# ETHZ-RobotX/open3d_slam_advanced_rss_2024_public

Hardware: AMD Instinct MI355X
Metric: ICP iterations/s (100k-pt scan vs 2M-pt map) (higher is better)
Workload: dtype f32; 1 GPU; C2: 100000-pt scan vs 2000000-pt voxel map, 0.1 m voxels, 50 iters, icp.yaml chain (KDTree maxDist 0.5 exact, Trimmed 0.9, SurfaceNormal 1.57, PointToPlane); scan_points=100000, map_points=2000000, pairs_per_gpu=1, parallelism=1 independent scan/map pair, 1 per GPU, no data-path collective

## Files before the change

### open3d_slam_advanced_rss_2024_public_amd/csrc/icp_kernels.h

```cpp
#pragma once
#include <hip/hip_runtime.h>
#include <math.h>
#include <stdint.h>
#include "host_post.h"
#include "icp_types.h"
#include "solve_device.h"

#pragma clang fp contract(off)

namespace o3s {
namespace kern {

constexpr int kBlock = 256;

constexpr float kInfF = __builtin_huge_valf();

template <int CTRL>
__device__ __forceinline__ int dpp_i32(int v) {
  return __builtin_amdgcn_update_dpp(v, v, CTRL, 0xF, 0xF, false);
}
template <int CTRL>
__device__ __forceinline__ double dpp_f64(double v) {
  const int lo = dpp_i32<CTRL>(__double2loint(v)), hi = dpp_i32<CTRL>(__double2hiint(v));
  return __hiloint2double(hi, lo);
}
__device__ __forceinline__ double readlane_f64(double v, int lane) {
// ... 403 lines not shown
  uint32_t tot;
  uint32_t ex = block_excl_scan(s, &tot, sh) + sums[blockIdx.x];
#pragma unroll
  for (int k = 0; k < kScanItems; ++k) {
    if (base + k < n) out[base + k] = ex;
    ex += v[k];
  }
  if (base <= n - 1 && n - 1 < base + kScanItems) out[n] = ex;
}

constexpr int kMaxQTiles = 2048;
constexpr int kTileReplicas = 8;
__device__ __forceinline__ uint32_t qcount_slot(uint32_t lin) { return (lin & ~2047u) | ((lin & 63u) << 5) | ((lin >> 6) & 31u); }
static_assert(kScanTile == 2048, "qcount_slot transposes a 64 x 32 tile");
struct Mat16 {
  float v[16];
};
struct PrepInit {
  uint32_t* hist;
  int hist_words;
  uint32_t* sel;
  int sel_words;
  float4* mq;
  float* cert;
  IcpState* state;
  int seed_differential;
  uint32_t seq;
};

__global__ void __launch_bounds__(kBlock) k_read_prep(const float4* __restrict__ in_xyzw, const float* __restrict__ in_n ,
                                                      int N, Mat16 T0, GridParams g,
                                                      float* __restrict__ tx, float* __restrict__ ty, float* __restrict__ tz,
                                                      float* __restrict__ tnx, float* __restrict__ tny, float* __restrict__ tnz,
                                                      uint32_t* __restrict__ cell_of, uint32_t* __restrict__ counts ,
                                                      int qf, int qnx, int qny, PrepInit init,
                                                      uint32_t* __restrict__ ticket ,
                                                      uint32_t* __restrict__ tile_cnt ,
                                                      int32_t* __restrict__ perm ) {
  const int i = blockIdx.x * kBlock + threadIdx.x;
  if (init.hist) {
    const int stride = gridDim.x * kBlock;
    for (int k = i; k < init.hist_words; k += stride) init.hist[k] = 0u;
    for (int k = i; k < init.sel_words; k += stride) init.sel[k] = 0u;
    if (blockIdx.x == 0) {
      constexpr int kWords = (int)(sizeof(IcpState) / 4);
      uint32_t* w = reinterpret_cast<uint32_t*>(init.state);
      for (int k = threadIdx.x; k < kWords; k += kBlock) w[k] = 0u;
      __syncthreads();
      if (threadIdx.x == 0) {
        IcpState* S = init.state;
        S->T_iter[0] = S->T_iter[5] = S->T_iter[10] = S->T_iter[15] = 1.f;
        S->limit = kInfF;
        S->call_seq = init.seq;
        S->t_prep = wall_clock64();
        if (init.seed_differential) {
          S->quat_ring[0][3] = 1.f;
          S->hist_total = 1;
        }
      }
    }
  }
  __shared__ uint32_t s_tile[kMaxQTiles];
  if (counts) {
    for (int k = threadIdx.x; k < kMaxQTiles; k += kBlock) s_tile[k] = 0u;
    __syncthreads();
  }
  int my_tile = -1;
  if (i < N) {
    if (init.mq) init.mq[i] = make_float4(0.f, 0.f, 0.f, 0.f);
    if (init.cert) init.cert[i] = 0.f;
    const float4 p = in_xyzw[i];
    float T[16];
#pragma unroll
    for (int k = 0; k < 16; ++k) T[k] = T0.v[k];
    const float x = xf_row(T, 0, p.x, p.y, p.z), y = xf_row(T, 1, p.x, p.y, p.z), z = xf_row(T, 2, p.x, p.y, p.z);
    tx[i] = x;
    ty[i] = y;
    tz[i] = z;
    if (in_n) {
      const float a = in_n[3 * i], b = in_n[3 * i + 1], c = in_n[3 * i + 2];
      tnx[i] = rot_row(T, 0, a, b, c);
      tny[i] = rot_row(T, 1, a, b, c);
      tnz[i] = rot_row(T, 2, a, b, c);
    }
    if (counts) {
      const int cx = cell_coord(x, g.ox, g.inv_cell, g.nx);
      const int cy = cell_coord(y, g.oy, g.inv_cell, g.ny);
      const int cz = cell_coord(z, g.oz, g.inv_cell, g.nz);
      const uint32_t lin = ((uint32_t)(cz / qf) * (uint32_t)qny + (uint32_t)(cy / qf)) * (uint32_t)qnx + (uint32_t)(cx / qf);
      cell_of[i] = lin;
      ticket[i] = atomicAdd(&counts[qcount_slot(lin)], 1u);
      const int tile = (int)(lin / (uint32_t)kScanTile);
      if (atomicAdd(&s_tile[tile], 1u) == 0u) my_tile = tile;
// ... 196 lines not shown
    d = c ? od : d;
    idx = c ? oi : idx;
  }
  gd = d;
  gi = idx;
}

constexpr int kFarMaxCells = 4096;

constexpr int kFarWaves = 5;
constexpr int kFarQ = 6;
template <bool STATS, int G, int UN, int RCB, bool FAR, bool CERT>
__global__ void __launch_bounds__(kBlock, FAR ? kFarWaves : 7) k_match2(const float* __restrict__ rx, const float* __restrict__ ry, const float* __restrict__ rz,
                                                      int N, const float4* __restrict__ ref, const uint32_t* __restrict__ cell_start,
                                                      GridParams g, IcpState* __restrict__ st,
                                                      int32_t* __restrict__ pos_out, float* __restrict__ d2_out, float4* __restrict__ mq,
                                                      uint32_t* __restrict__ hist_rep,
                                                      const float4* __restrict__ refn ,
                                                      float4* __restrict__ mn ,
                                                      const float* __restrict__ rnx, const float* __restrict__ rny,
                                                      const float* __restrict__ rnz ,
                                                      int rep_mask ,
                                                      uint32_t* __restrict__ spec ,
                                                      float* __restrict__ cert
                                                      O3S_DBG_PARAM
                                                      O3S_HOOK_PARAM(uint32_t* __restrict__ settled_cnt )) {
  __shared__ uint32_t s_hist[kHistBins];
  __shared__ uint32_t s_cnt[2];
  if (threadIdx.x < 2) s_cnt[threadIdx.x] = 0u;
#ifdef O3S_TEST_HOOKS
  __shared__ uint32_t s_set[2];
  if (threadIdx.x < 2) s_set[threadIdx.x] = 0u;
#endif
  constexpr int TQ = kBlock / G;
  constexpr int NK = (9 + G - 1) / G;
  const int sub = threadIdx.x & (G - 1);
  const int qib = threadIdx.x / G;
  const int tile = (blockIdx.x & 7) * (gridDim.x >> 3) + (blockIdx.x >> 3);
  const int i = tile * TQ + qib;
  const bool valid = i < N;
  const float hv = hdr_load(st);
  const float hp = CERT ? reinterpret_cast<const float*>(st->T_prev)[threadIdx.x & 31] : 0.f;
  float px = 0.f, py = 0.f, pz = 0.f;
  float4 inc = make_float4(0.f, 0.f, 0.f, 0.f);
  float cq = 0.f;
  int pe = -1;
  if (valid) {
    px = rx[i];
    py = ry[i];
    pz = rz[i];
    inc = mq[i];
    if (CERT) {
      cq = cert[i];
      pe = pos_out[i];
    }
  }
  for (int k = threadIdx.x; k < kHistBins; k += kBlock) s_hist[k] = 0u;
  if (hdr_i(hv, H_DONE)) return;
  if (blockIdx.x == 0) {
    for (int k = threadIdx.x; k < 1024; k += kBlock) hist_rep[(size_t)kHistReplicas * kHistBins + k] = 0u;
    if (threadIdx.x == 0 && hdr_i(hv, H_ITER) == 0) st->t_begin = wall_clock64();
    if (spec)
      for (int k = threadIdx.x; k < kSpecHalf; k += kBlock) spec[(size_t)((hdr_i(hv, H_ITER) + 1) & 1) * kSpecHalf + k] = 0u;
    if (CERT && threadIdx.x == 0) st->cert_seq[hdr_i(hv, H_ITER) & 1] = (uint32_t)hdr_i(hv, H_ITER) + 1u;
  }
  const uint32_t hint = __float_as_uint(hdr_f(hv, H_LIMIT));
  const bool spec_on = spec != nullptr && hdr_i(hv, H_ITER) > 0 && hint < 0x7f800000u;
  uint32_t* const spec_cur = spec_on ? spec + (size_t)(hdr_i(hv, H_ITER) & 1) * kSpecHalf : nullptr;
  float T[16];
#pragma unroll
  for (int k = 0; k < 16; ++k) T[k] = hdr_f(hv, k);
  __syncthreads();
  const float lim = g.max_r2;
  unsigned long long n_cand = 0, n_rows = 0;

  const float sx = xf_row(T, 0, px, py, pz), sy = xf_row(T, 1, px, py, pz), sz = xf_row(T, 2, px, py, pz);
// ... 2 lines not shown
  int gi = 0x7fffffff;
  bool active = valid && ((fabsf(sx) + fabsf(sy)) + fabsf(sz) < kInfF);
  float bound = lim;
  int mybin = -1;
  auto count_match = [&](float d) {
    const int bin = (int)((__float_as_uint(d) >> 20) & (kHistBins - 1));
    if (!O3S_DBG(1) && atomicAdd(&s_hist[bin], 1u) == 0u) mybin = bin;
    if (spec_on && !O3S_DBG(1)) {
      const uint32_t key = __float_as_uint(d) & 0x7fffffffu;
      if ((key >> 20) == (hint >> 20)) atomicAdd(&spec_cur[(key >> 10) & 1023u], 1u);
      if ((key >> 10) == (hint >> 10)) atomicAdd(&spec_cur[1024 + (key & 1023u)], 1u);
    }
  };
  uint32_t n_found = 0u, n_below = 0u;
  auto tally = [&](bool counted, float d) {
    if (spec_on && !O3S_DBG(1)) {
      const bool below = counted && ((__float_as_uint(d) & 0x7fffffffu) >> 20) < (hint >> 20);
      n_found += (uint32_t)__popcll(__ballot(counted));
      n_below += (uint32_t)__popcll(__ballot(below));
    }
  };
  bool wave_settled = false;
  bool settled = false;
  if (CERT) {
    float Tp[16];
#pragma unroll
    for (int k = 0; k < 16; ++k) Tp[k] = hdr_f(hp, k);
    float dn = 0.f, cn = 0.f;
    const bool fresh = (uint32_t)hdr_i(hp, 16 + ((hdr_i(hv, H_ITER) + 1) & 1)) == (uint32_t)hdr_i(hv, H_ITER);
    if (fresh && active && cq > 0.f) {
      const float ex = sx - xf_row(Tp, 0, px, py, pz), ey = sy - xf_row(Tp, 1, px, py, pz), ez = sz - xf_row(Tp, 2, px, py, pz);
      const float delta = __builtin_sqrtf((ex * ex + ey * ey) + ez * ez) * (1.f + 1e-6f);
      const float L = __builtin_sqrtf(cq) - delta;
      const float L2 = L * L, thr = L2 * (1.f - 1e-5f);
      cn = L2 * (1.f - 1e-6f);
      if (inc.w != 0.f) {
        dn = dist2(sx, sy, sz, inc.x, inc.y, inc.z);
        settled = (L > 0.f) & (pe != -1) & (dn <= lim) & (dn < thr);
      } else {
        settled = (L > 0.f) & (thr > lim);
      }
    }
    wave_settled = __all(!valid || settled);
#ifdef O3S_TEST_HOOKS
    if (settled_cnt && hdr_i(hv, H_ITER) < kSpecTrace) {
      const int n_set = __popcll(__ballot(settled && sub == 0));
      if ((threadIdx.x & 63) == 0 && n_set) {
        atomicAdd(&s_set[0], (uint32_t)n_set);
        if (wave_settled) atomicAdd(&s_set[1], (uint32_t)n_set);
      }
    }
#endif
    if (settled && !O3S_DBG(8)) {
      if (sub == 0) {
        if (inc.w != 0.f) {
          pos_out[i] = pe >= 0 ? pe : -2 - pe;
          d2_out[i] = dn;
          count_match(dn);
        }
        cert[i] = cn;
      }
    }
    tally(settled && !O3S_DBG(8) && sub == 0 && inc.w != 0.f, dn);
    active = active && !settled;
  }
  if (active) {
    const float di = dist2(sx, sy, sz, inc.x, inc.y, inc.z);
    bound = ((inc.w != 0.f) & (di <= lim)) ? di : lim;
  }
  float others = kInfF;
  auto group_cert = [&](float o) {
    float cn = (gi != 0x7fffffff && b.idx == gi) ? o : fminf(o, b.d);
    if (G >= 2) cn = fminf(cn, __int_as_float(dpp_i32<0xB1>(__float_as_int(cn))));
    if (G >= 4) cn = fminf(cn, __int_as_float(dpp_i32<0x4E>(__float_as_int(cn))));
    return ((fabsf(sx) + fabsf(sy)) + fabsf(sz) < kInfF) ? cn * (1.f - 1e-6f) : 0.f;
  };
  if (FAR && rnx != nullptr && lim * g.inv_cell * g.inv_cell >= 25.f && !wave_settled && __any(valid && !settled && inc.w == 0.f)) {
    constexpr int kProbeSteps = 12;
    constexpr int NP = (2 * kProbeSteps + G - 1) / G;
    const bool want = valid && !settled && inc.w == 0.f;
    float nx = 0.f, ny = 0.f, nz = 0.f;
    if (want) {
      const float a = rnx[i], b_ = rny[i], c_ = rnz[i];
      nx = rot_row(T, 0, a, b_, c_);
      ny = rot_row(T, 1, a, b_, c_);
      nz = rot_row(T, 2, a, b_, c_);
    }
    const int n_steps = min(kProbeSteps, (int)(__builtin_sqrtf(lim) * g.inv_cell) + 1);
    U32Pair hd[NP];
    int kk_[NP];
#pragma unroll
    for (int u = 0; u < NP; ++u) {
      const int e = sub + u * G;
      const int st_ = (e >> 1) + 1;
      const float t_ = (float)st_ * g.cell * ((e & 1) ? -1.f : 1.f);
      const float qx_ = sx + t_ * nx, qy_ = sy + t_ * ny, qz_ = sz + t_ * nz;
      const int cx_ = (int)floorf((qx_ - g.ox) * g.inv_cell), cy_ = (int)floorf((qy_ - g.oy) * g.inv_cell), cz_ = (int)floorf((qz_ - g.oz) * g.inv_cell);
      const bool in = want & (st_ <= n_steps) & ((unsigned)cx_ < (unsigned)g.nx) & ((unsigned)cy_ < (unsigned)g.ny) & ((unsigned)cz_ < (unsigned)g.nz);
// ... 24 lines not shown
    if (G >= 2) ds = fminf(ds, __int_as_float(dpp_i32<0xB1>(__float_as_int(ds))));
    if (G >= 4) ds = fminf(ds, __int_as_float(dpp_i32<0x4E>(__float_as_int(ds))));
    bound = fminf(bound, ds);
  }
  if (active) {
    const CellGeom c = cell_geom(sx, sy, sz, g);
    const float gxn = fmaxf(c.lx - g.margin, 0.f), gxp = fmaxf((g.cell - c.lx) - g.margin, 0.f);
    const float gyn = fmaxf(c.ly - g.margin, 0.f), gyp = fmaxf((g.cell - c.ly) - g.margin, 0.f);
    const float gzn = fmaxf(c.lz - g.margin, 0.f), gzp = fmaxf((g.cell - c.lz) - g.margin, 0.f);
    const float gxn2 = gxn * gxn, gxp2 = gxp * gxp, gyn2 = gyn * gyn, gyp2 = gyp * gyp, gzn2 = gzn * gzn, gzp2 = gzp * gzp;
    uint32_t jb[NK], len[NK];
    {
      uint4 w[NK];
      int span[NK];
      uint32_t inm[NK];
#pragma unroll
      for (int k = 0; k < NK; ++k) {
        const int t = sub + k * G, tt = t < 9 ? t : 4;
        const int dz = tt / 3 - 1, dy = tt % 3 - 1;
        const int z = c.cz + dz, y = c.cy + dy;
        const float gz2 = dz < 0 ? gzn2 : (dz > 0 ? gzp2 : 0.f);
        const float gy2 = dy < 0 ? gyn2 : (dy > 0 ? gyp2 : 0.f);
        const float g2 = gz2 + gy2;
        const float rem = bound - g2;
        const bool lskip = gxn2 > rem, rskip = gxp2 > rem;
        const int lo = max(c.cx - (int)!lskip, 0);
        const int hi = min(c.cx + (int)!rskip, g.nx - 1);
        const bool row = (t < 9) & ((unsigned)y < (unsigned)g.ny) & ((unsigned)z < (unsigned)g.nz);
        const bool in = row & (lo <= hi) & !(g2 > bound) & !O3S_DBG(4);
        const float ol = (lskip & ((unsigned)(c.cx - 1) < (unsigned)g.nx)) ? g2 + gxn2 : kInfF;
        const float orr = (rskip & ((unsigned)(c.cx + 1) < (unsigned)g.nx)) ? g2 + gxp2 : kInfF;
        others = row ? fminf(others, (g2 > bound) ? g2 : fminf(ol, orr)) : others;
        inm[k] = (uint32_t) - (int)in;
        span[k] = hi - lo;
        const uint32_t off = (((uint32_t)z * (uint32_t)g.ny + (uint32_t)y) * (uint32_t)g.nx + (uint32_t)lo) & inm[k];
        w[k] = *reinterpret_cast<const uint4*>(cell_start + off);
      }
#pragma unroll
      for (int k = 0; k < NK; ++k) {
        const uint32_t ve = span[k] == 0 ? w[k].y : (span[k] == 1 ? w[k].z : w[k].w);
        jb[k] = w[k].x & inm[k];
        len[k] = (ve - w[k].x) & inm[k];
        if (STATS) {
          n_rows += len[k] ? 1 : 0;
          n_cand += (unsigned long long)len[k];
        }
      }
    }
    uint32_t P[9], D[9];
    uint32_t total = 0;
#pragma unroll
    for (int t = 0; t < 9; ++t) {
      const uint32_t l_t = group_bcast_dyn<G>(len[t / G], t % G);
      const uint32_t j_t = group_bcast_dyn<G>(jb[t / G], t % G);
      P[t] = total;
// ... 5 lines not shown
      float4 qv[UN];
      uint32_t jj[UN];
      bool ok[UN];
#pragma unroll
      for (int u = 0; u < UN; ++u) {
        const uint32_t f = f0 + (uint32_t)(u * G);
        ok[u] = f < total;
        uint32_t dsel = D[0];
#pragma unroll
        for (int t = 1; t < 9; ++t) dsel = (P[t] <= f) ? D[t] : dsel;
        jj[u] = ok[u] ? f + dsel : 0u;
        qv[u] = ref[jj[u]];
      }
#pragma unroll
      for (int u = 0; u < UN; ++u) own_take(b, others, dist2(sx, sy, sz, qv[u].x, qv[u].y, qv[u].z), qv[u], (int)jj[u], lim, ok[u]);
    }
  }
  group_min_di<G>(b.d, b.idx, gd, gi);
  {
    const float q = g.cell - g.margin;
    const bool far = active && !(q * q > fminf(gd, bound)) && !O3S_DBG(16);
    if (active && !far) others = fminf(others, q * q);
    if (!FAR && CERT && valid && !settled && !O3S_DBG(8)) {
      const float cn = group_cert(far ? 0.f : others);
      if (sub == 0) cert[i] = cn;
    }
    active = far;
  }
  if (FAR) {
    if (__any(active)) {
      constexpr int Q = kFarQ;
      const CellGeom c = cell_geom(sx, sy, sz, g);
      const float m_yz = fminf(fminf(c.ly, g.cell - c.ly), fminf(c.lz, g.cell - c.lz));
      const int rho0 = max(max(0, max(-c.cy, c.cy - (g.ny - 1))), max(-c.cz, c.cz - (g.nz - 1)));
      const int rho_max = max(max(c.cy, g.ny - 1 - c.cy), max(c.cz, g.nz - 1 - c.cz));
      int rho = rho0;
      float best = fminf(gd, bound);
      auto ring_lb2_yz = [&](int r) {
        const float lb = (float)(r - 1) * g.cell + m_yz - g.margin;
        return (r >= 2 && lb > 0.f) ? lb * lb : 0.f;
      };
      if (active && rho <= rho_max && ring_lb2_yz(rho) > best) others = fminf(others, ring_lb2_yz(rho));
      if (rho > rho_max || ring_lb2_yz(rho) > best) active = false;
      uint32_t qa[Q], qb[Q];
#pragma unroll
      for (int k = 0; k < Q; ++k) qa[k] = qb[k] = 0u;
      while (__any(active)) {
// ... 173 lines not shown
#pragma unroll
                for (int v = 0; v < RCB; ++v) q[v] = ref[j + v < j1 ? j + v : j0];
#pragma unroll
                for (int v = 0; v < RCB; ++v) own_take(b, no_cert, dist2(sx, sy, sz, q[v].x, q[v].y, q[v].z), q[v], (int)(j + v), lim, j + v < j1);
              }
              if (STATS) {
                n_rows += j1 > j0 ? 1 : 0;
                n_cand += (unsigned long long)(j1 - j0);
              }
            }
          }
        }
      }
      group_min_di<G>(b.d, b.idx, gd, gi);
      if (active) {
        r += 1;
        if (r > rmax || ring_lb2(r, m, g) + extra2 > fminf(gd, bound)) active = false;
      }
    }
  }
  bool counted = false;
  if (valid && !settled && !O3S_DBG(8)) {
    const bool found = gi != 0x7fffffff;
    const float cn = (FAR && CERT) ? group_cert(others) : 0.f;
    bool mine = found && b.idx == gi && b.pos >= 0;
    if (FAR && G >= 2) {
      const uint32_t m = mine ? 1u : 0u;
      const uint32_t m0 = group_bcast<G, 0>(m), m1 = group_bcast<G, 1 % G>(m), m2 = group_bcast<G, 2 % G>(m);
      const bool lower = ((sub > 0) & (m0 != 0u)) | ((G >= 4) & (sub > 1) & (m1 != 0u)) | ((G >= 4) & (sub > 2) & (m2 != 0u));
      mine = mine && !lower;
    }
    if (mine) {
      const float4 nq = (mn && refn) ? refn[b.pos] : make_float4(0.f, 0.f, 0.f, 0.f);
      pos_out[i] = b.pos;
      d2_out[i] = b.d;
      mq[i] = make_float4(b.qx, b.qy, b.qz, 1.f);
      if (mn) mn[i] = nq;
      if (FAR && CERT) cert[i] = cn;
      count_match(b.d);
      counted = true;
    } else if (!found && sub == 0) {
      pos_out[i] = -1;
      d2_out[i] = kInfF;
      mq[i] = make_float4(0.f, 0.f, 0.f, 0.f);
      if (mn) mn[i] = make_float4(0.f, 0.f, 0.f, 0.f);
      if (FAR && CERT) cert[i] = cn;
    }
// ... 1395 lines not shown
  float p[3], q[3];
  const float4 nn = mn[i];
  cov_chain_pair(T, rx[i], ry[i], rz[i], mq[i], st->mp[0], st->mp[1], st->mp[2], st->mq[0], st->mq[1], st->mq[2], p, q);
  float* o = out + (size_t)i * 9;
  o[0] = p[0], o[1] = p[1], o[2] = p[2], o[3] = q[0], o[4] = q[1], o[5] = q[2], o[6] = nn.x, o[7] = nn.y, o[8] = nn.z;
  keep[i] = k ? 1 : 0;
}

__global__ void __launch_bounds__(kBlock) k_export_matches(int N, const int32_t* __restrict__ pos, const float* __restrict__ d2,
                                                           const float4* __restrict__ ref, const int32_t* __restrict__ perm,
                                                           int32_t* __restrict__ ids, float* __restrict__ dists) {
  const int i = blockIdx.x * kBlock + threadIdx.x;
  if (i >= N) return;
  const int pe = pos[i];
  const int o = perm[i];
  const int slot = pe >= 0 ? pe : (pe <= -2 ? -2 - pe : -1);
  ids[o] = slot >= 0 ? __float_as_int(ref[slot].w) : -1;
  dists[o] = d2[i];
}

__global__ void __launch_bounds__(kBlock) k_import_matches(int N, const int32_t* __restrict__ ids, const float* __restrict__ dists,
                                                           const float* __restrict__ weights , const int32_t* __restrict__ orig_to_sorted,
                                                           int64_t M, const float4* __restrict__ ref, int32_t* __restrict__ pos, float* __restrict__ d2,
                                                           float4* __restrict__ mq, float* __restrict__ cert ) {
  const int i = blockIdx.x * kBlock + threadIdx.x;
  if (i >= N) return;
  if (cert) cert[i] = 0.f;
  const int id = ids[i];
  const float d = dists[i];
  int pe = -1;
  if (id >= 0 && (int64_t)id < M) {
    pe = orig_to_sorted[id];
    if (weights && weights[i] == 0.0f) pe = -2 - pe;
  }
  float4 q = make_float4(0.f, 0.f, 0.f, 0.f);
  if (id >= 0 && (int64_t)id < M) {
    const float4 r = ref[orig_to_sorted[id]];
    q = make_float4(r.x, r.y, r.z, 1.f);
  }
  mq[i] = q;
  if (d == kInfF) pe = pe >= 0 ? -2 - pe : pe;
  pos[i] = pe;
  d2[i] = d;
}

__global__ void __launch_bounds__(kBlock) k_weights(int N, const int32_t* __restrict__ pos, const float* __restrict__ d2,
                                                    const float* __restrict__ read_n , const float4* __restrict__ refn,
                                                    ChainParams cp, const IcpState* __restrict__ st, int any_filter, float* __restrict__ w) {
  const int i = blockIdx.x * kBlock + threadIdx.x;
  if (i >= N) return;
// ... 37 lines not shown
```

### open3d_slam_advanced_rss_2024_public_amd/csrc/icp_types.h

```cpp
#pragma once
#include <stddef.h>
#include <stdint.h>
#include <hip/hip_runtime.h>

#ifdef O3S_TEST_HOOKS
#include <stdlib.h>
#define O3S_HOOK_ENV(name) getenv(name)
#define O3S_DBG_PARAM , int dbg
#define O3S_DBG_ARG(x) , (x)
#define O3S_HOOK_PARAM(decl) , decl
#define O3S_DBG(bits) ((dbg & (bits)) != 0)
#define O3S_CP_DBG(cp, bits) (((cp).dbg & (bits)) != 0)
#else
#define O3S_HOOK_ENV(name) ((const char*)0)
#define O3S_DBG_PARAM
#define O3S_DBG_ARG(x)
#define O3S_HOOK_PARAM(decl)
#define O3S_DBG(bits) false
#define O3S_CP_DBG(cp, bits) false
#endif

namespace o3s {

constexpr int kHistBins = 2048;
// ... 57 lines not shown
  float point_used_ratio, weighted_ratio;
  float A[36];
  float b[6];
  float x[6];
  float dT[16];
  float ang_ring[kHistRing];
  float tnorm_ring[kHistRing];
  uint32_t call_seq;
  uint32_t posted;
  unsigned long long t_begin;
  unsigned long long t_end;
  unsigned long long t_prep;
  unsigned long long cand_count;
  unsigned long long row_count;
  float T_prev[16];
  uint32_t cert_seq[2];
  uint32_t tail_pad[14];
};
constexpr int kStateWords = (int)(offsetof(IcpState, T_prev) / 4);
constexpr int kStateTailWords = 4;
static_assert(offsetof(IcpState, T_prev) == offsetof(IcpState, row_count) + 8, "the staged words end with the matcher's counters");
static_assert(sizeof(IcpState) % 4 == 0, "IcpState is copied word-wise");
static_assert(offsetof(IcpState, cert_seq) == offsetof(IcpState, T_prev) + 64 && sizeof(IcpState) == offsetof(IcpState, T_prev) + 128,
              "k_match2 loads T_prev and cert_seq as one 32-word block");

struct CandRec {
  float px, py, pz;
  uint32_t bits;
  float qx, qy, qz;
  int32_t keep;
};

struct SelScratch {
  uint32_t seg_count[kSegs];
  uint32_t bin;
  uint32_t kk;
  uint32_t bin_count;
  uint32_t skip;
  uint32_t reserved;
  uint32_t pad[3];
  uint32_t depth;
  uint32_t limit_bits;
  uint32_t pad2[2];
};
static_assert(sizeof(SelScratch) == 64, "the selection kernels read the hand-off words one per lane (lanes 0..15)");
constexpr int kSelWordDepth = 12, kSelWordLimit = 13;

// ... 10 lines not shown
```

### open3d_slam_advanced_rss_2024_public_amd/csrc/o3s_icp.hip

```cpp
#include "../../include/o3s_icp.h"

#include <hip/hip_runtime.h>

#include <algorithm>
#include <cmath>
#include <cstdio>
#include <cstdlib>
#include <cstring>
#include <limits>
#include <string>
#include <vector>

#include "icp_kernels.h"
#include "icp_shard_kernels.h"
#include "icp_types.h"

#pragma clang fp contract(off)

using namespace o3s;

namespace {

thread_local std::string g_create_error;

// ... 29 lines not shown
struct HostStage {
  IcpState state;
  IcpState eval_state;
  float T0[16];
  double ref_part[1024 * 3];
  float ref_bb[1024 * 6];
  uint32_t n_occ;
};

constexpr int kNumKernels = 5;
constexpr size_t kCovBufBytes = ((size_t)kMaxPartialBlocks * kCovComps + kCovComps + 3) * sizeof(double);
static_assert(kCovBufBytes >= (2 * (size_t)kern::kFitMaxBlocks + 4) * sizeof(double), "k_fit's block partials and its four totals fit the covariance pass's area");
constexpr size_t kHistWords = (size_t)kHistReplicas * kHistBins + 1024;
constexpr size_t kHookTraceWords = (1 + 2 * (size_t)kHistReplicas) * kSpecTrace;

struct ChainArgs {
  int N;
  int match_g;
  int nb_match, nb_part, nb_cls;
  int nb_fused;
  bool has_n;
  uint32_t* spec;
  int no_bin_counters;
  float* cert;
  float *rx, *ry, *rz, *rnx, *rny, *rnz;
  ChainParams cp;
  GridParams g;
};

struct Call {
  bool live = false;
  ChainArgs a{};
  bool stats = false;
  float Tc[16], T0[16];
  int iters_cap = 0;
  enum Issue { kEager, kReplay, kProfiled } issue = kEager;
  int first = 0, step = 0;
  int issued = 0;
  bool ends_inside() const { return a.cp.max_iters > 0 && issued >= a.cp.max_iters; }
};

}

struct o3s_icp {
  o3s_icp_config cfg;
  int device = 0;
  hipStream_t own_stream = nullptr, stream = nullptr;
// ... 371 lines not shown
    h->qcells = (size_t)h->qnx * (size_t)h->qny * (size_t)h->qnz;
  }
  HIP_TRY(h, h->d_qstart.ensure((h->qcells + 1) * 4));
  if (wait_end) HIP_TRY(h, hipStreamSynchronize(h->stream));
  h->M = M;
  h->ref_has_normals = d_normals != nullptr;
  h->ref_ready = true;
  h->reading_ready = false;
  if (h->graph_exec) {
    (void)hipGraphExecDestroy(h->graph_exec);
    h->graph_exec = nullptr;
  }
  return O3S_OK;
}

int ensure_iteration_buffers(o3s_icp* h, int N) {
  HIP_TRY(h, h->d_t.ensure((size_t)N * 6 * 4));
  HIP_TRY(h, h->d_r.ensure((size_t)N * 6 * 4));
  HIP_TRY(h, h->d_perm.ensure((size_t)N * 4));
  HIP_TRY(h, h->d_qcell.ensure((size_t)N * 4));
  HIP_TRY(h, h->d_pos.ensure((size_t)N * 4));
  HIP_TRY(h, h->d_d2.ensure((size_t)N * 4));
  HIP_TRY(h, h->d_mq.ensure((size_t)N * sizeof(float4)));
  HIP_TRY(h, h->d_cert.ensure((size_t)N * 4));
  HIP_TRY(h, h->d_mn.ensure((size_t)N * sizeof(float4)));
  HIP_TRY(h, h->d_hist.ensure((kHistWords + kSpecWords + kHookTraceWords) * 4));
  HIP_TRY(h, h->d_cand.ensure((size_t)nblocks(N, kern::kClsBlock) * kern::kClsBlock * sizeof(CandRec)));
  HIP_TRY(h, h->d_cand_cnt.ensure(((size_t)nblocks(N, kern::kClsBlock) * 2 + 2) * 4));
  HIP_TRY(h, h->d_sel.ensure(sizeof(SelScratch)));
  HIP_TRY(h, h->d_sel_part2.ensure((size_t)kCentComps * kern::kSelPartMaxBlocks * sizeof(double)));
  HIP_TRY(h, h->d_park.ensure((size_t)kern::kParkRecs * (sizeof(CandRec) + 4)));
  HIP_TRY(h, h->d_cent.ensure((size_t)nblocks(N) * kCentComps * sizeof(double)));
  HIP_TRY(h, h->d_ne.ensure((size_t)kMaxPartialBlocks * kNeComps * sizeof(double)));
  HIP_TRY(h, h->d_state.ensure(sizeof(IcpState)));
  HIP_TRY(h, h->d_T0.ensure(16 * 4));
  if (h->cfg.error_minimizer == 1) HIP_TRY(h, h->d_cov.ensure(kCovBufBytes));
  return O3S_OK;
}

int ensure_qcount(o3s_icp* h) {
  const size_t words = ((h->qcells + kern::kScanTile - 1) / kern::kScanTile) * kern::kScanTile + (size_t)kern::kMaxQTiles * kern::kTileReplicas;
  const size_t cap_before = h->d_qcount.cap;
  HIP_TRY(h, h->d_qcount.ensure(words * 4));
  if (h->d_qcount.cap != cap_before) HIP_TRY(h, hipMemsetAsync(h->d_qcount.p, 0, h->d_qcount.cap, h->stream));
  return O3S_OK;
}

// ... 14 lines not shown
  a.nb_cls = nblocks(h->N, kern::kClsBlock);
  a.nb_part = std::min(kMaxPartialBlocks, nblocks(h->N, kern::kBlock * kern::kNePPT));
  if (h->shard.active) {
    const int64_t per_rank = (h->shard.n_total + h->shard.world - 1) / h->shard.world;
    a.nb_part = std::min(kMaxPartialBlocks, nblocks(per_rank, kern::kBlock * kern::kNePPT));
  }
  {
    const char* fe = O3S_HOOK_ENV("O3S_FUSE");
    const bool fuse = !(fe && std::atoi(fe) == 0);
    const int nbf = nblocks(h->N, kern::kBlock * kern::kNePPT);
    a.nb_fused = (fuse && !h->shard.active && !h->many_in_flight && nbf <= kern::kFusedMaxBlocks && nbf == a.nb_part) ? nbf : 0;
  }
  a.has_n = h->read_has_normals;
  {
    const char* ne = O3S_HOOK_ENV("O3S_NO_SPEC_SELECT");
    const bool spec = cp.has_trim && !cp.mirror && !h->shard.active && !(ne && std::atoi(ne) != 0);
    a.spec = spec ? h->d_hist.as<uint32_t>() + kHistWords : nullptr;
    const char* nb = O3S_HOOK_ENV("O3S_NO_BIN_COUNTERS");
    a.no_bin_counters = (nb && std::atoi(nb) != 0) ? 1 : 0;
  }
  {
    const char* nc = O3S_HOOK_ENV("O3S_NO_CERT");
    const bool on = !cp.mirror && !h->shard.active && !(nc && std::atoi(nc) != 0) && !O3S_CP_DBG(cp, ~0);
    a.cert = on ? h->d_cert.as<float>() : nullptr;
  }
  float* r = h->d_r.as<float>();
  a.rx = r;
  a.ry = r + (size_t)h->N;
  a.rz = r + 2 * (size_t)h->N;
  a.rnx = r + 3 * (size_t)h->N;
  a.rny = r + 4 * (size_t)h->N;
  a.rnz = r + 5 * (size_t)h->N;
  a.cp = cp;
  a.g = h->grid;
  return a;
}

uint32_t* chain_hist(o3s_icp* h) {
  return h->shard.active ? reinterpret_cast<uint32_t*>(h->shard.xbuf + kXchgI32Off) : h->d_hist.as<uint32_t>();
}
int chain_replicas(const o3s_icp* h) { return h->shard.active ? shard_replicas(h->shard.world) : kHistReplicas; }

inline bool normals_from_matcher(const ChainArgs& a) { return a.N >= 200000 && !a.cp.mirror; }
struct RefIndex {
  const float4* ref;
  const float4* refn;
  const uint32_t* cell_start;
  GridParams g;
};
inline bool first_index_used(const o3s_icp* h, const ChainParams& cp) { return !cp.mirror && h->have_grid1 && h->far_rows; }
inline RefIndex main_index(o3s_icp* h) { return RefIndex{h->d_ref.as<float4>(), h->d_refn.as<float4>(), h->d_cell_start.as<uint32_t>(), h->grid}; }
inline RefIndex chain_index(o3s_icp* h, const ChainParams& cp, int it) {
  if (it == 0 && first_index_used(h, cp))
    return RefIndex{h->d_ref1.as<float4>(), h->ref_has_normals ? h->d_refn1.as<float4>() : h->d_refn.as<float4>(), h->d_cell_start1.as<uint32_t>(), h->grid1};
  return main_index(h);
}
template <bool STATS, int G, bool CERT>
void launch_match2(o3s_icp* h, const ChainArgs& a, const ChainParams& cp, const RefIndex& ix, uint32_t* spec, float* cert, hipStream_t s) {
#ifdef O3S_TEST_HOOKS
  uint32_t* const settled = CERT ? h->d_hist.as<uint32_t>() + kHistWords + kSpecWords + kSpecTrace : nullptr;
#endif
  const int nb = round_up8(nblocks(a.N, kern::kBlock / G));
  if (h->far_rows)
    hipLaunchKernelGGL((kern::k_match2<STATS, G, 2, 4, true, CERT>), dim3(nb), dim3(kern::kBlock), 0, s, a.rx, a.ry, a.rz, a.N, ix.ref, ix.cell_start, ix.g,
                       h->d_state.as<IcpState>(), h->d_pos.as<int32_t>(), h->d_d2.as<float>(), h->d_mq.as<float4>(), chain_hist(h), ix.refn,
                       normals_from_matcher(a) ? h->d_mn.as<float4>() : (float4*)nullptr, a.has_n ? a.rnx : (const float*)nullptr, a.rny, a.rnz,
                       chain_replicas(h) - 1, spec, CERT ? cert : (float*)nullptr O3S_DBG_ARG(cp.dbg) O3S_DBG_ARG(settled));
  else
    hipLaunchKernelGGL((kern::k_match2<STATS, G, 2, 2, false, CERT>), dim3(nb), dim3(kern::kBlock), 0, s, a.rx, a.ry, a.rz, a.N, ix.ref, ix.cell_start, ix.g,
                       h->d_state.as<IcpState>(), h->d_pos.as<int32_t>(), h->d_d2.as<float>(), h->d_mq.as<float4>(), chain_hist(h), ix.refn,
                       normals_from_matcher(a) ? h->d_mn.as<float4>() : (float4*)nullptr, a.has_n ? a.rnx : (const float*)nullptr, a.rny, a.rnz,
                       chain_replicas(h) - 1, spec, CERT ? cert : (float*)nullptr O3S_DBG_ARG(cp.dbg) O3S_DBG_ARG(settled));
}
inline int match_lanes(const o3s_icp* h, const ChainArgs& a, bool first) {
  return (first && h->far_rows && a.N < 200000) ? 4 : a.match_g;
}
void launch_match2_any(o3s_icp* h, const ChainArgs& a, const ChainParams& cp, bool stats, bool first, const RefIndex& ix, uint32_t* spec, float* cert,
                       hipStream_t s) {
  if (cp.mirror) {
    hipLaunchKernelGGL(kern::k_match_mirror, dim3(nblocks(a.N)), dim3(kern::kBlock), 0, s, a.N, h->d_ref.as<float4>(), h->d_orig_to_sorted.as<int32_t>(),
                       h->d_perm.as<int32_t>(), h->d_state.as<IcpState>(), h->d_pos.as<int32_t>(), h->d_d2.as<float>(), h->d_mq.as<float4>(),
                       chain_hist(h));
    return;
  }
  const int G = match_lanes(h, a, first);
  auto go = [&](auto st_, auto g_) {
    if (cert) launch_match2<decltype(st_)::value, decltype(g_)::value, true>(h, a, cp, ix, spec, cert, s);
    else launch_match2<decltype(st_)::value, decltype(g_)::value, false>(h, a, cp, ix, spec, cert, s);
  };
  using std::integral_constant;
  if (stats) {
    if (G == 2) go(std::true_type{}, integral_constant<int, 2>{});
    else go(std::true_type{}, integral_constant<int, 4>{});
  } else {
    if (G == 2) go(std::false_type{}, integral_constant<int, 2>{});
    else go(std::false_type{}, integral_constant<int, 4>{});
  }
}
void launch_match_any(o3s_icp* h, const ChainArgs& a, const ChainParams& cp, bool stats, hipStream_t s, bool first = false) {
  launch_match2_any(h, a, cp, stats, first, main_index(h), nullptr, nullptr, s);
}
void launch_match_chain(o3s_icp* h, const ChainArgs& a, bool stats, hipStream_t s, int it, const RefIndex& ix) {
  float* const cert = it == 0 ? nullptr : a.cert;
  launch_match2_any(h, a, a.cp, stats, it == 0, ix, a.spec, cert, s);
}

inline bool sel_partial(const ChainArgs& a) {
  const char* pe = O3S_HOOK_ENV("O3S_SEL_PARTIAL");
  return a.nb_cls > kern::kFinThreads && !(pe && std::atoi(pe) == 0);
}

void launch_iteration(o3s_icp* h, const ChainArgs& a, bool stats, hipEvent_t* ev , int it) {
  IcpState* st = h->d_state.as<IcpState>();
  hipStream_t s = h->stream;
  const int mode = kern::kModeCentroid | kern::kModeGate | (normals_from_matcher(a) ? kern::kModeNormalReady : 0);
  if (ev) (void)hipEventRecord(ev[0], s);
  const RefIndex ix = chain_index(h, a.cp, it);
  launch_match_chain(h, a, stats, s, it, ix);
  if (ev) (void)hipEventRecord(ev[1], s);
  hipLaunchKernelGGL(kern::k_classify, dim3(a.nb_cls), dim3(kern::kClsBlock), 0, s, a.rx, a.ry, a.rz, a.rnx, a.rny, a.rnz, a.N, ix.ref,
                     ix.refn, h->d_pos.as<int32_t>(), h->d_d2.as<float>(), h->d_hist.as<uint32_t>(), a.cp, st,
                     h->d_sel.as<SelScratch>(), h->d_cand.as<CandRec>(), h->d_cand_cnt.as<uint32_t>(), h->d_hist.as<uint32_t>() + (size_t)kHistReplicas * kHistBins, h->d_mq.as<float4>(), h->d_mn.as<float4>(), h->d_cent.as<double>(), mode, kHistReplicas,
                     10, 1023u, a.spec, a.cp.mirror ? kern::kInfF : ix.g.max_r2 O3S_DBG_ARG(a.no_bin_counters));
  if (ev) (void)hipEventRecord(ev[2], s);
  uint32_t* hist2 = h->d_hist.as<uint32_t>() + (size_t)kHistReplicas * kHistBins;
  if (a.nb_fused > 0) {
// ... 74 lines not shown

bool graph_key_equal(const o3s_icp::GraphKey& a, const o3s_icp::GraphKey& b) {
  return a.N == b.N && a.iters == b.iters && a.nb == b.nb && a.has_n == b.has_n && a.gen == b.gen && std::memcmp(a.ptrs, b.ptrs, sizeof(a.ptrs)) == 0 &&
         std::memcmp(&a.cp, &b.cp, sizeof(ChainParams)) == 0 && std::memcmp(&a.g, &b.g, sizeof(GridParams)) == 0 && a.have_grid1 == b.have_grid1 &&
         std::memcmp(&a.g1, &b.g1, sizeof(GridParams)) == 0;
}

int prepare_reading(o3s_icp* h, const float* T0, bool sort, bool reset_chain, bool seed_differential) {
  const int N = h->N;
  const float4* in = reinterpret_cast<const float4*>(h->ext_xyzw ? h->ext_xyzw : h->d_in_xyzw.p);
  const float* in_n = h->read_has_normals ? reinterpret_cast<const float*>(h->ext_n ? h->ext_n : h->d_in_n.p) : nullptr;
  kern::Mat16 T0v;
  std::memcpy(T0v.v, T0, 16 * sizeof(float));
  kern::PrepInit init{};
  if (reset_chain) {
    init.hist = chain_hist(h);
    init.hist_words = h->shard.active ? (int)(kXchgL1Words + kShardL2Bins) : (int)kHistWords;
#ifdef O3S_TEST_HOOKS
    if (!h->shard.active) init.hist_words += (int)(kSpecWords + kHookTraceWords);
#endif
    init.sel = h->d_sel.as<uint32_t>();
    init.sel_words = (int)(sizeof(SelScratch) / 4);
    init.mq = h->d_mq.as<float4>();
    init.cert = h->d_cert.as<float>();
    init.state = h->d_state.as<IcpState>();
    init.seed_differential = seed_differential ? 1 : 0;
    init.seq = h->call_seq;
  }
  float* t = h->d_t.as<float>();
  float* r = h->d_r.as<float>();
  const size_t n = (size_t)N;
  const int nb = nblocks(N);
  if (sort) {
    const int n_tiles = (int)((h->qcells + kern::kScanTile - 1) / kern::kScanTile);
    int rc = ensure_qcount(h);
    if (rc != O3S_OK) return rc;
    uint32_t* counts = h->d_qcount.as<uint32_t>();
    uint32_t* tile_cnt = counts + (size_t)n_tiles * kern::kScanTile;
    uint32_t* ticket = h->d_d2.as<uint32_t>();
    hipLaunchKernelGGL(kern::k_read_prep, dim3(nb), dim3(kern::kBlock), 0, h->stream, in, in_n, N, T0v, h->grid, t, t + n,
                       t + 2 * n, t + 3 * n, t + 4 * n, t + 5 * n, h->d_qcell.as<uint32_t>(), counts, h->qf, h->qnx,
                       h->qny, init, ticket, tile_cnt, (int32_t*)nullptr);
    hipLaunchKernelGGL(kern::k_read_starts, dim3(n_tiles), dim3(kern::kBlock), 0, h->stream, counts, (int64_t)h->qcells, tile_cnt,
                       h->d_qstart.as<uint32_t>());
    const char* so = O3S_HOOK_ENV("O3S_SCATTER_ORDER");
    int32_t* who = h->d_pos.as<int32_t>();
    hipLaunchKernelGGL(kern::k_read_scatter, dim3(nb), dim3(kern::kBlock), 0, h->stream, N, h->d_qcell.as<uint32_t>(), h->d_qstart.as<uint32_t>(),
// ... 978 lines not shown
  HIP_TRY(h, h->d_mod_a.ensure((size_t)N * 4));
  HIP_TRY(h, h->d_mod_b.ensure((size_t)N * 4));
  hipLaunchKernelGGL(kern::k_export_matches, dim3(nblocks(N)), dim3(kern::kBlock), 0, h->stream, (int)N, h->d_pos.as<int32_t>(),
                     h->d_d2.as<float>(), h->d_ref.as<float4>(), h->d_perm.as<int32_t>(), h->d_mod_a.as<int32_t>(), h->d_mod_b.as<float>());
  HIP_TRY(h, hipGetLastError());
  HIP_TRY(h, hipMemcpyAsync(ids, h->d_mod_a.p, (size_t)N * 4, hipMemcpyDeviceToHost, h->stream));
  HIP_TRY(h, hipMemcpyAsync(dists2, h->d_mod_b.p, (size_t)N * 4, hipMemcpyDeviceToHost, h->stream));
  HIP_TRY(h, hipStreamSynchronize(h->stream));
  h->reading_ready = false;
  return O3S_OK;
}

static int import_matches(o3s_icp* h, const int32_t* ids, const float* dists2, const float* weights, int64_t N) {
  HIP_TRY(h, h->d_mod_a.ensure((size_t)N * 4));
  HIP_TRY(h, h->d_mod_b.ensure((size_t)N * 4));
  HIP_TRY(h, hipMemcpyAsync(h->d_mod_a.p, ids, (size_t)N * 4, hipMemcpyHostToDevice, h->stream));
  HIP_TRY(h, hipMemcpyAsync(h->d_mod_b.p, dists2, (size_t)N * 4, hipMemcpyHostToDevice, h->stream));
  if (weights) {
    HIP_TRY(h, h->d_mod_c.ensure((size_t)N * 4));
    HIP_TRY(h, hipMemcpyAsync(h->d_mod_c.p, weights, (size_t)N * 4, hipMemcpyHostToDevice, h->stream));
  }
  hipLaunchKernelGGL(kern::k_import_matches, dim3(nblocks(N)), dim3(kern::kBlock), 0, h->stream, (int)N, h->d_mod_a.as<int32_t>(),
                     h->d_mod_b.as<float>(), weights ? h->d_mod_c.as<float>() : (const float*)nullptr, h->d_orig_to_sorted.as<int32_t>(), h->M,
                     h->d_ref.as<float4>(), h->d_pos.as<int32_t>(), h->d_d2.as<float>(), h->d_mq.as<float4>(), h->d_cert.as<float>());
  HIP_TRY(h, hipGetLastError());
  return O3S_OK;
}

int o3s_icp_outlier_weights(o3s_icp* h, const float* reading_normals, const int32_t* ids, const float* dists2, int64_t N, float* weights) {
  if (!h || !ids || !dists2 || !weights) return O3S_ERR_BAD_ARGUMENT;
  if (!h->ref_ready) return fail(h, O3S_ERR_NOT_INITIALIZED, "outlier_weights before a successful init_reference");
  if (N <= 0) return fail(h, O3S_ERR_EMPTY_READING, "empty matches");
  h->elements_valid = false;
  HIP_TRY(h, hipSetDevice(h->device));
  int rc = ensure_iteration_buffers(h, (int)N);
  if (rc != O3S_OK) return rc;
  h->reading_ready = false;
  rc = import_matches(h, ids, dists2, nullptr, N);
  if (rc != O3S_OK) return rc;
  ChainParams cp = make_chain(h, reading_normals != nullptr);
  const bool any = h->cfg.trim_ratio >= 0.f || h->cfg.max_normal_angle >= 0.f || h->cfg.max_dist_outlier >= 0.f;
  IcpState st0;
  init_state(st0);
  rc = push_state(h, st0);
  if (rc != O3S_OK) return rc;
  HIP_TRY(h, hipMemsetAsync(h->d_hist.p, 0, kHistWords * 4, h->stream));
  HIP_TRY(h, hipMemsetAsync(h->d_sel.p, 0, sizeof(SelScratch), h->stream));
// ... 163 lines not shown
```

Measured before the change: 34220 ICP iterations/s.

## Store transformed point in certificate and widen search for near-settled queries

The per-point certificate grows from a float to a float4 that also holds the transformed query position from the previous iteration. Point drift is now taken directly from that stored position instead of reapplying the previous transform loaded from state, and settled points no longer rewrite their certificate. A new 'thin' case, for points that barely moved but did not settle, widens the search bound by a constant factor capped at the limit, so the certificate written this iteration is more likely to let the point settle next time. This trades four times the certificate memory traffic, plus a larger search for thin points, for fewer full neighbour searches.

```diff
diff --git a/open3d_slam_advanced_rss_2024_public_amd/csrc/cert_settle.h b/open3d_slam_advanced_rss_2024_public_amd/csrc/cert_settle.h
--- /dev/null
+++ b/open3d_slam_advanced_rss_2024_public_amd/csrc/cert_settle.h
@@ -0,0 +1,25 @@
+#pragma once
+
+#if defined(__HIPCC__) || defined(__CUDACC__)
+#define O3S_CERT_HD __host__ __device__ __forceinline__
+#else
+#define O3S_CERT_HD inline
+#endif
+
+namespace o3s {
+
+O3S_CERT_HD float cert_scale(float others_min) { return others_min * (1.f - 1e-6f); }
+
+O3S_CERT_HD bool cert_settles(float c, float ex, float ey, float ez, bool matched, bool has_slot, float dn, float max_r2) {
+  if (!(c > 0.f)) return false;
+  const float delta = __builtin_sqrtf((ex * ex + ey * ey) + ez * ez) * (1.f + 1e-6f);
+  const float L = __builtin_sqrtf(c) - delta;
+  const float thr = (L * L) * (1.f - 1e-5f);
+  return matched ? ((L > 0.f) & has_slot & (dn <= max_r2) & (dn < thr)) : ((L > 0.f) & (thr > max_r2));
+}
+
+O3S_CERT_HD bool cert_thin(float c, float ex, float ey, float ez) { return (c > 0.f) & ((ex * ex + ey * ey) + ez * ez < 1e-4f * c); }
+
+constexpr float kCertWiden = 1.21f;
+
+}
diff --git a/open3d_slam_advanced_rss_2024_public_amd/csrc/icp_kernels.h b/open3d_slam_advanced_rss_2024_public_amd/csrc/icp_kernels.h
--- a/open3d_slam_advanced_rss_2024_public_amd/csrc/icp_kernels.h
+++ b/open3d_slam_advanced_rss_2024_public_amd/csrc/icp_kernels.h
@@ -2,6 +2,7 @@
 #include <hip/hip_runtime.h>
 #include <math.h>
 #include <stdint.h>
+#include "cert_settle.h"
 #include "host_post.h"
 #include "icp_types.h"
 #include "solve_device.h"
@@ -451,7 +452,7 @@
   uint32_t* sel;
   int sel_words;
   float4* mq;
-  float* cert;
+  float4* cert;
   IcpState* state;
   int seed_differential;
   uint32_t seq;
@@ -497,7 +498,7 @@
   int my_tile = -1;
   if (i < N) {
     if (init.mq) init.mq[i] = make_float4(0.f, 0.f, 0.f, 0.f);
-    if (init.cert) init.cert[i] = 0.f;
+    if (init.cert) init.cert[i] = make_float4(0.f, 0.f, 0.f, 0.f);
     const float4 p = in_xyzw[i];
     float T[16];
 #pragma unroll
@@ -740,7 +741,7 @@
                                                       const float* __restrict__ rnz ,
                                                       int rep_mask ,
                                                       uint32_t* __restrict__ spec ,
-                                                      float* __restrict__ cert
+                                                      float4* __restrict__ cert
                                                       O3S_DBG_PARAM
                                                       O3S_HOOK_PARAM(uint32_t* __restrict__ settled_cnt )) {
   __shared__ uint32_t s_hist[kHistBins];
@@ -758,10 +759,10 @@
   const int i = tile * TQ + qib;
   const bool valid = i < N;
   const float hv = hdr_load(st);
-  const float hp = CERT ? reinterpret_cast<const float*>(st->T_prev)[threadIdx.x & 31] : 0.f;
+  const uint32_t hq = CERT ? st->cert_seq[threadIdx.x & 1] : 0u;
   float px = 0.f, py = 0.f, pz = 0.f;
   float4 inc = make_float4(0.f, 0.f, 0.f, 0.f);
-  float cq = 0.f;
+  float4 cr = make_float4(0.f, 0.f, 0.f, 0.f);
   int pe = -1;
   if (valid) {
     px = rx[i];
@@ -769,7 +770,7 @@
     pz = rz[i];
     inc = mq[i];
     if (CERT) {
-      cq = cert[i];
+      cr = cert[i];
       pe = pos_out[i];
     }
   }
@@ -818,24 +819,16 @@
   };
   bool wave_settled = false;
   bool settled = false;
+  bool thin = false;
   if (CERT) {
-    float Tp[16];
-#pragma unroll
-    for (int k = 0; k < 16; ++k) Tp[k] = hdr_f(hp, k);
-    float dn = 0.f, cn = 0.f;
-    const bool fresh = (uint32_t)hdr_i(hp, 16 + ((hdr_i(hv, H_ITER) + 1) & 1)) == (uint32_t)hdr_i(hv, H_ITER);
-    if (fresh && active && cq > 0.f) {
-      const float ex = sx - xf_row(Tp, 0, px, py, pz), ey = sy - xf_row(Tp, 1, px, py, pz), ez = sz - xf_row(Tp, 2, px, py, pz);
-      const float delta = __builtin_sqrtf((ex * ex + ey * ey) + ez * ez) * (1.f + 1e-6f);
-      const float L = __builtin_sqrtf(cq) - delta;
-      const float L2 = L * L, thr = L2 * (1.f - 1e-5f);
-      cn = L2 * (1.f - 1e-6f);
-      if (inc.w != 0.f) {
-        dn = dist2(sx, sy, sz, inc.x, inc.y, inc.z);
-        settled = (L > 0.f) & (pe != -1) & (dn <= lim) & (dn < thr);
-      } else {
-        settled = (L > 0.f) & (thr > lim);
-      }
+    float dn = 0.f;
+    const bool fresh = (uint32_t)__builtin_amdgcn_readlane((int)hq, (hdr_i(hv, H_ITER) + 1) & 1) == (uint32_t)hdr_i(hv, H_ITER);
+    if (fresh && active && cr.w > 0.f) {
+      const float ex = sx - cr.x, ey = sy - cr.y, ez = sz - cr.z;
+      const bool matched = inc.w != 0.f;
+      dn = matched ? dist2(sx, sy, sz, inc.x, inc.y, inc.z) : 0.f;
+      settled = cert_settles(cr.w, ex, ey, ez, matched, pe != -1, dn, lim);
+      thin = !settled && cert_thin(cr.w, ex, ey, ez);
     }
     wave_settled = __all(!valid || settled);
 #ifdef O3S_TEST_HOOKS
@@ -848,13 +841,10 @@
     }
 #endif
     if (settled && !O3S_DBG(8)) {
-      if (sub == 0) {
-        if (inc.w != 0.f) {
-          pos_out[i] = pe >= 0 ? pe : -2 - pe;
-          d2_out[i] = dn;
-          count_match(dn);
-        }
-        cert[i] = cn;
+      if (sub == 0 && inc.w != 0.f) {
+        pos_out[i] = pe >= 0 ? pe : -2 - pe;
+        d2_out[i] = dn;
+        count_match(dn);
       }
     }
     tally(settled && !O3S_DBG(8) && sub == 0 && inc.w != 0.f, dn);
@@ -864,12 +854,13 @@
     const float di = dist2(sx, sy, sz, inc.x, inc.y, inc.z);
     bound = ((inc.w != 0.f) & (di <= lim)) ? di : lim;
   }
+  const float bound_open = (CERT && thin) ? fminf(kCertWiden * bound, lim) : bound;
   float others = kInfF;
   auto group_cert = [&](float o) {
     float cn = (gi != 0x7fffffff && b.idx == gi) ? o : fminf(o, b.d);
     if (G >= 2) cn = fminf(cn, __int_as_float(dpp_i32<0xB1>(__float_as_int(cn))));
     if (G >= 4) cn = fminf(cn, __int_as_float(dpp_i32<0x4E>(__float_as_int(cn))));
-    return ((fabsf(sx) + fabsf(sy)) + fabsf(sz) < kInfF) ? cn * (1.f - 1e-6f) : 0.f;
+    return make_float4(sx, sy, sz, ((fabsf(sx) + fabsf(sy)) + fabsf(sz) < kInfF) ? cert_scale(cn) : 0.f);
   };
   if (FAR && rnx != nullptr && lim * g.inv_cell * g.inv_cell >= 25.f && !wave_settled && __any(valid && !settled && inc.w == 0.f)) {
     constexpr int kProbeSteps = 12;
@@ -940,15 +931,15 @@
         const float gz2 = dz < 0 ? gzn2 : (dz > 0 ? gzp2 : 0.f);
         const float gy2 = dy < 0 ? gyn2 : (dy > 0 ? gyp2 : 0.f);
         const float g2 = gz2 + gy2;
-        const float rem = bound - g2;
+        const float rem = bound_open - g2;
         const bool lskip = gxn2 > rem, rskip = gxp2 > rem;
         const int lo = max(c.cx - (int)!lskip, 0);
         const int hi = min(c.cx + (int)!rskip, g.nx - 1);
         const bool row = (t < 9) & ((unsigned)y < (unsigned)g.ny) & ((unsigned)z < (unsigned)g.nz);
-        const bool in = row & (lo <= hi) & !(g2 > bound) & !O3S_DBG(4);
+        const bool in = row & (lo <= hi) & !(g2 > bound_open) & !O3S_DBG(4);
         const float ol = (lskip & ((unsigned)(c.cx - 1) < (unsigned)g.nx)) ? g2 + gxn2 : kInfF;
         const float orr = (rskip & ((unsigned)(c.cx + 1) < (unsigned)g.nx)) ? g2 + gxp2 : kInfF;
-        others = row ? fminf(others, (g2 > bound) ? g2 : fminf(ol, orr)) : others;
+        others = row ? fminf(others, (g2 > bound_open) ? g2 : fminf(ol, orr)) : others;
         inm[k] = (uint32_t) - (int)in;
         span[k] = hi - lo;
         const uint32_t off = (((uint32_t)z * (uint32_t)g.ny + (uint32_t)y) * (uint32_t)g.nx + (uint32_t)lo) & inm[k];
@@ -1000,7 +991,7 @@
     const bool far = active && !(q * q > fminf(gd, bound)) && !O3S_DBG(16);
     if (active && !far) others = fminf(others, q * q);
     if (!FAR && CERT && valid && !settled && !O3S_DBG(8)) {
-      const float cn = group_cert(far ? 0.f : others);
+      const float4 cn = group_cert(far ? 0.f : others);
       if (sub == 0) cert[i] = cn;
     }
     active = far;
@@ -1220,7 +1211,7 @@
   bool counted = false;
   if (valid && !settled && !O3S_DBG(8)) {
     const bool found = gi != 0x7fffffff;
-    const float cn = (FAR && CERT) ? group_cert(others) : 0.f;
+    const float4 cn = (FAR && CERT) ? group_cert(others) : make_float4(0.f, 0.f, 0.f, 0.f);
     bool mine = found && b.idx == gi && b.pos >= 0;
     if (FAR && G >= 2) {
       const uint32_t m = mine ? 1u : 0u;
@@ -2662,10 +2653,10 @@
 __global__ void __launch_bounds__(kBlock) k_import_matches(int N, const int32_t* __restrict__ ids, const float* __restrict__ dists,
                                                            const float* __restrict__ weights , const int32_t* __restrict__ orig_to_sorted,
                                                            int64_t M, const float4* __restrict__ ref, int32_t* __restrict__ pos, float* __restrict__ d2,
-                                                           float4* __restrict__ mq, float* __restrict__ cert ) {
+                                                           float4* __restrict__ mq, float4* __restrict__ cert ) {
   const int i = blockIdx.x * kBlock + threadIdx.x;
   if (i >= N) return;
-  if (cert) cert[i] = 0.f;
+  if (cert) cert[i] = make_float4(0.f, 0.f, 0.f, 0.f);
   const int id = ids[i];
   const float d = dists[i];
   int pe = -1;
diff --git a/open3d_slam_advanced_rss_2024_public_amd/csrc/icp_types.h b/open3d_slam_advanced_rss_2024_public_amd/csrc/icp_types.h
--- a/open3d_slam_advanced_rss_2024_public_amd/csrc/icp_types.h
+++ b/open3d_slam_advanced_rss_2024_public_amd/csrc/icp_types.h
@@ -103,7 +103,7 @@
 static_assert(offsetof(IcpState, T_prev) == offsetof(IcpState, row_count) + 8, "the staged words end with the matcher's counters");
 static_assert(sizeof(IcpState) % 4 == 0, "IcpState is copied word-wise");
 static_assert(offsetof(IcpState, cert_seq) == offsetof(IcpState, T_prev) + 64 && sizeof(IcpState) == offsetof(IcpState, T_prev) + 128,
-              "k_match2 loads T_prev and cert_seq as one 32-word block");
+              "T_prev and cert_seq share one 128-byte line behind the staged words");
 
 struct CandRec {
   float px, py, pz;
diff --git a/open3d_slam_advanced_rss_2024_public_amd/csrc/o3s_icp.hip b/open3d_slam_advanced_rss_2024_public_amd/csrc/o3s_icp.hip
--- a/open3d_slam_advanced_rss_2024_public_amd/csrc/o3s_icp.hip
+++ b/open3d_slam_advanced_rss_2024_public_amd/csrc/o3s_icp.hip
@@ -75,7 +75,7 @@
   bool has_n;
   uint32_t* spec;
   int no_bin_counters;
-  float* cert;
+  float4* cert;
   float *rx, *ry, *rz, *rnx, *rny, *rnz;
   ChainParams cp;
   GridParams g;
@@ -493,7 +493,7 @@
   HIP_TRY(h, h->d_pos.ensure((size_t)N * 4));
   HIP_TRY(h, h->d_d2.ensure((size_t)N * 4));
   HIP_TRY(h, h->d_mq.ensure((size_t)N * sizeof(float4)));
-  HIP_TRY(h, h->d_cert.ensure((size_t)N * 4));
+  HIP_TRY(h, h->d_cert.ensure((size_t)N * 16));
   HIP_TRY(h, h->d_mn.ensure((size_t)N * sizeof(float4)));
   HIP_TRY(h, h->d_hist.ensure((kHistWords + kSpecWords + kHookTraceWords) * 4));
   HIP_TRY(h, h->d_cand.ensure((size_t)nblocks(N, kern::kClsBlock) * kern::kClsBlock * sizeof(CandRec)));
@@ -554,7 +554,7 @@
   {
     const char* nc = O3S_HOOK_ENV("O3S_NO_CERT");
     const bool on = !cp.mirror && !h->shard.active && !(nc && std::atoi(nc) != 0) && !O3S_CP_DBG(cp, ~0);
-    a.cert = on ? h->d_cert.as<float>() : nullptr;
+    a.cert = on ? h->d_cert.as<float4>() : nullptr;
   }
   float* r = h->d_r.as<float>();
   a.rx = r;
@@ -588,7 +588,7 @@
   return main_index(h);
 }
 template <bool STATS, int G, bool CERT>
-void launch_match2(o3s_icp* h, const ChainArgs& a, const ChainParams& cp, const RefIndex& ix, uint32_t* spec, float* cert, hipStream_t s) {
+void launch_match2(o3s_icp* h, const ChainArgs& a, const ChainParams& cp, const RefIndex& ix, uint32_t* spec, float4* cert, hipStream_t s) {
 #ifdef O3S_TEST_HOOKS
   uint32_t* const settled = CERT ? h->d_hist.as<uint32_t>() + kHistWords + kSpecWords + kSpecTrace : nullptr;
 #endif
@@ -597,17 +597,17 @@
     hipLaunchKernelGGL((kern::k_match2<STATS, G, 2, 4, true, CERT>), dim3(nb), dim3(kern::kBlock), 0, s, a.rx, a.ry, a.rz, a.N, ix.ref, ix.cell_start, ix.g,
                        h->d_state.as<IcpState>(), h->d_pos.as<int32_t>(), h->d_d2.as<float>(), h->d_mq.as<float4>(), chain_hist(h), ix.refn,
                        normals_from_matcher(a) ? h->d_mn.as<float4>() : (float4*)nullptr, a.has_n ? a.rnx : (const float*)nullptr, a.rny, a.rnz,
-                       chain_replicas(h) - 1, spec, CERT ? cert : (float*)nullptr O3S_DBG_ARG(cp.dbg) O3S_DBG_ARG(settled));
+                       chain_replicas(h) - 1, spec, CERT ? cert : (float4*)nullptr O3S_DBG_ARG(cp.dbg) O3S_DBG_ARG(settled));
   else
     hipLaunchKernelGGL((kern::k_match2<STATS, G, 2, 2, false, CERT>), dim3(nb), dim3(kern::kBlock), 0, s, a.rx, a.ry, a.rz, a.N, ix.ref, ix.cell_start, ix.g,
                        h->d_state.as<IcpState>(), h->d_pos.as<int32_t>(), h->d_d2.as<float>(), h->d_mq.as<float4>(), chain_hist(h), ix.refn,
                        normals_from_matcher(a) ? h->d_mn.as<float4>() : (float4*)nullptr, a.has_n ? a.rnx : (const float*)nullptr, a.rny, a.rnz,
-                       chain_replicas(h) - 1, spec, CERT ? cert : (float*)nullptr O3S_DBG_ARG(cp.dbg) O3S_DBG_ARG(settled));
+                       chain_replicas(h) - 1, spec, CERT ? cert : (float4*)nullptr O3S_DBG_ARG(cp.dbg) O3S_DBG_ARG(settled));
 }
 inline int match_lanes(const o3s_icp* h, const ChainArgs& a, bool first) {
   return (first && h->far_rows && a.N < 200000) ? 4 : a.match_g;
 }
-void launch_match2_any(o3s_icp* h, const ChainArgs& a, const ChainParams& cp, bool stats, bool first, const RefIndex& ix, uint32_t* spec, float* cert,
+void launch_match2_any(o3s_icp* h, const ChainArgs& a, const ChainParams& cp, bool stats, bool first, const RefIndex& ix, uint32_t* spec, float4* cert,
                        hipStream_t s) {
   if (cp.mirror) {
     hipLaunchKernelGGL(kern::k_match_mirror, dim3(nblocks(a.N)), dim3(kern::kBlock), 0, s, a.N, h->d_ref.as<float4>(), h->d_orig_to_sorted.as<int32_t>(),
@@ -633,7 +633,7 @@
   launch_match2_any(h, a, cp, stats, first, main_index(h), nullptr, nullptr, s);
 }
 void launch_match_chain(o3s_icp* h, const ChainArgs& a, bool stats, hipStream_t s, int it, const RefIndex& ix) {
-  float* const cert = it == 0 ? nullptr : a.cert;
+  float4* const cert = it == 0 ? nullptr : a.cert;
   launch_match2_any(h, a, a.cp, stats, it == 0, ix, a.spec, cert, s);
 }
 
@@ -754,7 +754,7 @@
     init.sel = h->d_sel.as<uint32_t>();
     init.sel_words = (int)(sizeof(SelScratch) / 4);
     init.mq = h->d_mq.as<float4>();
-    init.cert = h->d_cert.as<float>();
+    init.cert = h->d_cert.as<float4>();
     init.state = h->d_state.as<IcpState>();
     init.seed_differential = seed_differential ? 1 : 0;
     init.seq = h->call_seq;
@@ -1779,7 +1779,7 @@
   }
   hipLaunchKernelGGL(kern::k_import_matches, dim3(nblocks(N)), dim3(kern::kBlock), 0, h->stream, (int)N, h->d_mod_a.as<int32_t>(),
                      h->d_mod_b.as<float>(), weights ? h->d_mod_c.as<float>() : (const float*)nullptr, h->d_orig_to_sorted.as<int32_t>(), h->M,
-                     h->d_ref.as<float4>(), h->d_pos.as<int32_t>(), h->d_d2.as<float>(), h->d_mq.as<float4>(), h->d_cert.as<float>());
+                     h->d_ref.as<float4>(), h->d_pos.as<int32_t>(), h->d_d2.as<float>(), h->d_mq.as<float4>(), h->d_cert.as<float4>());
   HIP_TRY(h, hipGetLastError());
   return O3S_OK;
 }
```

Measured after the change: 34300 ICP iterations/s (median of 2 runs). No clear change (+0.2%).
